# EtherealEngine/Universal-Volumetric

Measured on AMD Instinct MI355X. Metric: frames/s encode, 100k-vert mesh + 2048^2 texture, higher is better.
Workload: dtype u8/int32 (f32 only in the quantiser)

## Files before the change

universal-volumetric_amd/csrc/tex_device.hpp:

```cpp
#pragma once
#include <hip/hip_runtime.h>
#include <cstdint>
#include "tex_blocks.hpp"

#define TEX_MAX_LAYERS 64
#define TEX_MAX_CODEBOOK 16128
#define TEX_HS 64
#define TEX_VQ_ROUNDS 24
#define TEX_NMODEL 9
#define TEX_MODEL_CAP (TEX_MAX_CODEBOOK + TEX_HS + 8)
#define TEX_E_ALPHA (-60)

struct TexVQ {
  uint32_t n_items, K, nl, done, m_round, round_active;
  uint32_t *leaf;
  unsigned long long *stW, *stS, *stQ;
  uint8_t *splittable, *chosen; int32_t *axis; long long *th, *prio; uint32_t *newidx;
  uint32_t *split;
};

struct TexHuff { uint32_t n; uint32_t *freq; uint8_t *size; uint16_t *code; };

struct TexJob {
  const uint8_t *layer[TEX_MAX_LAYERS];
  uint32_t W, H, L, bx, by, nb, NB;
  uint32_t ashift;
  int32_t yflip; uint32_t Kmax_e, Kmax_s, T_skip;
  int32_t status;
  uint8_t *skip;
  uint32_t *cell;
  uint32_t *hist;
  uint8_t *flag; uint32_t *bsum;
  uint32_t ncell; uint32_t *cid, *cw, *cidx;
  TexVQ vq[2];
  uint32_t *ent;
  uint32_t *ecb; uint32_t ne; uint32_t *emap;
  uint16_t *bei, *bsi; uint32_t *bsel;
  uint32_t n_items; uint32_t *item;
  uint32_t *scb; uint8_t *sused; uint32_t *scu; uint32_t ns; uint32_t *smap;
  uint8_t *pred;
  uint32_t *clist; uint32_t ncoded[TEX_MAX_LAYERS];
  uint8_t *msym; uint32_t *gid, *gstart, *gsize;
  unsigned long long *tok;
  TexHuff hm[TEX_NMODEL];
  uint32_t *hscratch;
  uint8_t *sec[3]; uint32_t sec_cap[3], sec_len[3];
  uint8_t *slice[TEX_MAX_LAYERS]; uint32_t slice_cap, slice_len[TEX_MAX_LAYERS];
  unsigned long long pack_off, pack_len;
  unsigned long long slice_bits[TEX_MAX_LAYERS];
  uint32_t n_skipped;
};

__device__ inline void t_load_block(const TexJob &J, uint32_t l, uint32_t X, uint32_t Y, uint32_t px[16], uint32_t *amask = nullptr) {
  const uint8_t *img = J.layer[l >> J.ashift];
  const bool akind = (l & J.ashift) != 0;
  for (int y = 0; y < 4; y++) {
    uint32_t py = Y * 4 + y; if (py >= J.H) py = J.H - 1;
    const uint32_t sr = J.yflip ? J.H - 1 - py : py;
    const uint8_t *row = img + 4 * ((size_t)sr * J.W);
    if (X * 4 + 3 < J.W && (J.W & 3) == 0) {
      const uint4 v = *reinterpret_cast<const uint4 *>(row + 16 * (size_t)X);
      if (akind) { px[4 * y + 0] = (v.x >> 24) * 0x010101u; px[4 * y + 1] = (v.y >> 24) * 0x010101u; px[4 * y + 2] = (v.z >> 24) * 0x010101u; px[4 * y + 3] = (v.w >> 24) * 0x010101u; }
      else { px[4 * y + 0] = v.x & 0xffffffu; px[4 * y + 1] = v.y & 0xffffffu; px[4 * y + 2] = v.z & 0xffffffu; px[4 * y + 3] = v.w & 0xffffffu; }
      if (amask) *amask &= v.x & v.y & v.z & v.w;
    } else {
      for (int x = 0; x < 4; x++) { uint32_t pxx = X * 4 + x; if (pxx >= J.W) pxx = J.W - 1; const uint8_t *p = row + 4 * (size_t)pxx; px[4 * y + x] = akind ? (uint32_t)p[3] * 0x010101u : ((uint32_t)p[0] | ((uint32_t)p[1] << 8) | ((uint32_t)p[2] << 16)); if (amask) *amask &= (uint32_t)p[3] << 24; }
    }
  }
}

template <bool WANT_SEL, bool WANT_ROWS>
__device__ inline uint32_t t_eval_block(const uint32_t px[16], int c5r, int c5g, int c5b, int t, uint32_t *sel_out, unsigned long long *rows) {
  const int br = t_expand5(c5r), bg = t_expand5(c5g), bb = t_expand5(c5b);
  int cr[4], cg[4], cb[4];
  for (int s = 0; s < 4; s++) { const int d = t_inten(t, s); cr[s] = t_clampi(br + d, 0, 255); cg[s] = t_clampi(bg + d, 0, 255); cb[s] = t_clampi(bb + d, 0, 255); }
  uint32_t tot = 0, sel = 0;
  if (!WANT_ROWS) {
    const int d0 = t_inten(t, 0), d1 = t_inten(t, 1), d2 = t_inten(t, 2), d3 = t_inten(t, 3);
    const int lo = br < bg ? (br < bb ? br : bb) : (bg < bb ? bg : bb), hi = br > bg ? (br > bb ? br : bb) : (bg > bb ? bg : bb);
    if (!WANT_SEL && lo + d0 >= 0 && hi + d3 <= 255) {
      const int kh = 3 * d3 * d3, kl = 3 * d2 * d2;
      for (int i = 0; i < 16; i++) {
        const int er = br - (int)(px[i] & 255), eg = bg - (int)((px[i] >> 8) & 255), eb = bb - (int)((px[i] >> 16) & 255);
        const int A = er * er + eg * eg + eb * eb, B2 = 2 * (er + eg + eb), ab = B2 < 0 ? -B2 : B2;
        const int a = kh - d3 * ab, b = kl - d2 * ab;
        tot += (uint32_t)(A + (a < b ? a : b));
      }
      return tot;
    }
    if (lo + d0 >= 0 && hi + d3 <= 255) {
      const int k0 = 3 * d0 * d0, k1 = 3 * d1 * d1, k2 = 3 * d2 * d2, k3 = 3 * d3 * d3;
      for (int i = 0; i < 16; i++) {
        const int er = br - (int)(px[i] & 255), eg = bg - (int)((px[i] >> 8) & 255), eb = bb - (int)((px[i] >> 16) & 255);
        const int A = er * er + eg * eg + eb * eb, B2 = 2 * (er + eg + eb);
        const uint32_t e0 = (uint32_t)(A + d0 * B2 + k0), e1 = (uint32_t)(A + d1 * B2 + k1), e2 = (uint32_t)(A + d2 * B2 + k2), e3 = (uint32_t)(A + d3 * B2 + k3);
        uint32_t be = e0; int bs = 0;
        if (e1 < be) { be = e1; bs = 1; }
        if (e2 < be) { be = e2; bs = 2; }
        if (e3 < be) { be = e3; bs = 3; }
        tot += be; sel |= (uint32_t)bs << (2 * i);
      }
      if (WANT_SEL) *sel_out = sel;
      return tot;
    }
  }
  for (int i = 0; i < 16; i++) {
    const int r = (int)(px[i] & 255), g = (int)((px[i] >> 8) & 255), b = (int)((px[i] >> 16) & 255);
    uint32_t be = 0xffffffffu; int bs = 0; unsigned long long row = 0;
    for (int s = 0; s < 4; s++) {
      const int dr = cr[s] - r, dg = cg[s] - g, db = cb[s] - b;
      const uint32_t e = (uint32_t)(dr * dr + dg * dg + db * db);
      if (WANT_ROWS) row |= (unsigned long long)(e > 65535u ? 65535u : e) << (16 * s);
      if (e < be) { be = e; bs = s; }
    }
    tot += be; sel |= (uint32_t)bs << (2 * i);
    if (WANT_ROWS) rows[i] = row;
  }
  if (WANT_SEL) *sel_out = sel;
  return tot;
}

#ifdef HIPEMU
__device__ inline void t_mfma_i8_16x16x64(const uint32_t a[4], const uint32_t b[4], int acc[4]) {
  const int lane = hipemu_lane(), col = lane & 15, rg = lane >> 4;
  const unsigned long long a01 = a[0] | ((unsigned long long)a[1] << 32), a23 = a[2] | ((unsigned long long)a[3] << 32);
  const unsigned long long b01 = b[0] | ((unsigned long long)b[1] << 32), b23 = b[2] | ((unsigned long long)b[3] << 32);
  bool ok;
  for (int g = 0; g < 4; g++) {
    const unsigned long long B0 = hipemu_wave_exchange(b01, col + 16 * g, &ok), B1 = hipemu_wave_exchange(b23, col + 16 * g, &ok);
    for (int r = 0; r < 4; r++) {
      const unsigned long long A0 = hipemu_wave_exchange(a01, 4 * rg + r + 16 * g, &ok), A1 = hipemu_wave_exchange(a23, 4 * rg + r + 16 * g, &ok);
      int sum = 0;
      for (int j = 0; j < 8; j++) sum += (int)(int8_t)(A0 >> (8 * j)) * (int)(int8_t)(B0 >> (8 * j)) + (int)(int8_t)(A1 >> (8 * j)) * (int)(int8_t)(B1 >> (8 * j));
      acc[r] += sum;
    }
  }
}
#else
typedef int t_v4i __attribute__((ext_vector_type(4)));
__device__ __forceinline__ void t_mfma_i8_16x16x64(const uint32_t a[4], const uint32_t b[4], int acc[4]) {
  const t_v4i va = { (int)a[0], (int)a[1], (int)a[2], (int)a[3] }, vb = { (int)b[0], (int)b[1], (int)b[2], (int)b[3] }, vc = { acc[0], acc[1], acc[2], acc[3] };
  const t_v4i vd = __builtin_amdgcn_mfma_i32_16x16x64_i8(va, vb, vc, 0, 0, 0);
  acc[0] = vd.x; acc[1] = vd.y; acc[2] = vd.z; acc[3] = vd.w;
}
#endif

__device__ __forceinline__ void t_cell_coords(uint32_t cell, int x[4]) {
  x[0] = t_expand5((cell >> 10) & 31); x[1] = t_expand5((cell >> 5) & 31); x[2] = t_expand5(cell & 31); x[3] = t_inten((cell >> 15) & 7, 3);
}

struct TBitW { uint8_t *p; uint32_t cap, n; unsigned long long acc; int nacc; int overflow; };
__device__ inline void tb_init(TBitW &w, uint8_t *p, uint32_t cap) { w.p = p; w.cap = cap; w.n = 0; w.acc = 0; w.nacc = 0; w.overflow = 0; }
__device__ inline void tb_put(TBitW &w, uint32_t v, int n) {
  while (n > 0) {
    const int k = n > 24 ? 24 : n;
    w.acc |= (unsigned long long)(v & ((1u << k) - 1)) << w.nacc; w.nacc += k; v >>= k; n -= k;
    while (w.nacc >= 8) { if (w.n < w.cap) w.p[w.n] = (uint8_t)(w.acc & 0xff); else w.overflow = 1; w.n++; w.acc >>= 8; w.nacc -= 8; }
  }
}
__device__ inline void tb_flush(TBitW &w) { if (w.nacc > 0) { if (w.n < w.cap) w.p[w.n] = (uint8_t)(w.acc & 0xff); else w.overflow = 1; w.n++; w.acc = 0; w.nacc = 0; } }

__device__ __forceinline__ void t_vlc(uint32_t v, int cb, unsigned long long &bits, int &len) {
  bits = 0; len = 0;
  for (;;) { const uint32_t chunk = v & ((1u << cb) - 1); v >>= cb; bits |= (unsigned long long)(chunk | (v ? (1u << cb) : 0u)) << len; len += cb + 1; if (!v) break; }
}
```

universal-volumetric_amd/csrc/tex_encode.hip:

```cpp
#include "uvol_common.hpp"
#include "tex_device.hpp"
#include <algorithm>

#define TJOB_OR_RETURN TexJob &J = job[blockIdx.z]; if (J.status != 0) return
#define TEX_RETRY_ALPHA (~(size_t)0)

__device__ inline uint32_t t_block_excl_scan(uint32_t v, uint32_t *total) {
  __shared__ uint32_t wsum[UVOL_BLOCK / 64];
  const int lane = threadIdx.x & 63, w = threadIdx.x >> 6;
  uint32_t x = v;
  for (int d = 1; d < 64; d <<= 1) { uint32_t y = __shfl_up(x, d); if (lane >= d) x += y; }
  if (lane == 63) wsum[w] = x;
  __syncthreads();
  uint32_t base = 0, tot = 0;
  for (int i = 0; i < UVOL_BLOCK / 64; i++) { if (i < w) base += wsum[i]; tot += wsum[i]; }
  __syncthreads();
  *total = tot;
  return base + x - v;
}
__global__ void __launch_bounds__(UVOL_BLOCK) k_tscan_a(TexJob *job, uint32_t n) {
  TexJob &J = job[blockIdx.z];
  const uint32_t i = blockIdx.x * UVOL_BLOCK + threadIdx.x;
  uint32_t v = (J.status == 0 && i < n) ? J.flag[i] : 0, tot;
  t_block_excl_scan(v, &tot);
  if (threadIdx.x == 0) J.bsum[blockIdx.x] = tot;
}
__global__ void __launch_bounds__(UVOL_BLOCK) k_tscan_b(TexJob *job, uint32_t nblocks) {
  TexJob &J = job[blockIdx.z];
  __shared__ uint32_t carry;
  if (threadIdx.x == 0) carry = 0;
  __syncthreads();
  for (uint32_t b0 = 0; b0 < nblocks; b0 += UVOL_BLOCK) {
    const uint32_t i = b0 + threadIdx.x;
    uint32_t v = i < nblocks ? J.bsum[i] : 0, tot;
    const uint32_t ex = t_block_excl_scan(v, &tot);
    const uint32_t c = carry;
    if (i < nblocks) J.bsum[i] = c + ex;
    __syncthreads();
    if (threadIdx.x == 0) carry = c + tot;
    __syncthreads();
  }
  if (threadIdx.x == 0) J.bsum[nblocks] = carry;
}

__global__ void __launch_bounds__(UVOL_BLOCK) k_tex_skip(TexJob *job) {
  TJOB_OR_RETURN;
  const uint32_t b = blockIdx.x * UVOL_BLOCK + threadIdx.x;
  if (b >= J.nb) return;
  const uint32_t X = b % J.bx, Y = b / J.bx;
  uint32_t anchor[16], cur[16], amask = 0xff000000u;
  const uint32_t st = 1u << J.ashift;
  for (uint32_t kind = 0; kind < st; kind++) {
    t_load_block(J, kind, X, Y, anchor, &amask);
    J.skip[(size_t)kind * J.nb + b] = 0; J.flag[(size_t)kind * J.nb + b] = 1;
    for (uint32_t l = kind + st; l < J.L; l += st) {
      t_load_block(J, l, X, Y, cur, &amask);
      uint32_t d = 0;
      for (int i = 0; i < 16; i++) {
        const int dr = (int)(cur[i] & 255) - (int)(anchor[i] & 255), dg = (int)((cur[i] >> 8) & 255) - (int)((anchor[i] >> 8) & 255), db = (int)((cur[i] >> 16) & 255) - (int)((anchor[i] >> 16) & 255);
        d += (uint32_t)(dr * dr + dg * dg + db * db);
      }
      const bool sk = d <= J.T_skip;
      J.skip[(size_t)l * J.nb + b] = sk ? 1 : 0; J.flag[(size_t)l * J.nb + b] = sk ? 0 : 1;
      if (!sk) for (int i = 0; i < 16; i++) anchor[i] = cur[i];
    }
  }
  if (!J.ashift && (amask & 0xff000000u) != 0xff000000u) J.status = TEX_E_ALPHA;
}

__global__ void __launch_bounds__(UVOL_BLOCK) k_tex_fit(TexJob *job) {
  TJOB_OR_RETURN;
  const uint32_t it = blockIdx.x * UVOL_BLOCK + threadIdx.x;
  if (it >= J.n_items) return;
  const uint32_t b = J.item[it];
  const uint32_t l = b / J.nb, r = b % J.nb;
  uint32_t px[16]; t_load_block(J, l, r % J.bx, r / J.bx, px);
  int sum[3] = {0, 0, 0};
  for (int i = 0; i < 16; i++) { sum[0] += (int)(px[i] & 255); sum[1] += (int)((px[i] >> 8) & 255); sum[2] += (int)((px[i] >> 16) & 255); }
  int base5[3]; for (int c = 0; c < 3; c++) base5[c] = (((sum[c] + 8) >> 4) * 31 + 127) / 255;
  uint32_t best = 0xffffffffu; int bc0 = 0, bc1 = 0, bc2 = 0, bt = 0;
  for (int t = 0; t < 8; t++) for (int di = 0; di < 3; di++) {
    const int dd = di == 0 ? 0 : (di == 1 ? -1 : 1);
    const int c0 = t_clampi(base5[0] + dd, 0, 31), c1 = t_clampi(base5[1] + dd, 0, 31), c2 = t_clampi(base5[2] + dd, 0, 31);
    const uint32_t e = t_eval_block<false, false>(px, c0, c1, c2, t, nullptr, nullptr);
    if (e < best) { best = e; bt = t; bc0 = c0; bc1 = c1; bc2 = c2; }
  }
  for (int c = 0; c < 3; c++) for (int di = 1; di < 3; di++) {
    const int dd = di == 1 ? -1 : 1;
    int c0 = bc0 + (c == 0 ? dd : 0), c1 = bc1 + (c == 1 ? dd : 0), c2 = bc2 + (c == 2 ? dd : 0);
    const int cc = c == 0 ? c0 : (c == 1 ? c1 : c2);
    if (cc < 0 || cc > 31) continue;
    const uint32_t e = t_eval_block<false, false>(px, c0, c1, c2, bt, nullptr, nullptr);
    if (e < best) { best = e; bc0 = c0; bc1 = c1; bc2 = c2; }
  }
  const uint32_t cell = ((uint32_t)bt << 15) | ((uint32_t)bc0 << 10) | ((uint32_t)bc1 << 5) | (uint32_t)bc2;
  J.cell[b] = cell;
  atomicAdd(&J.hist[cell], 1u);
}

__global__ void __launch_bounds__(UVOL_BLOCK) k_cell_flags(TexJob *job) {
  TJOB_OR_RETURN;
  const uint32_t c = blockIdx.x * UVOL_BLOCK + threadIdx.x;
  if (c < (1u << 18)) J.flag[c] = J.hist[c] ? 1 : 0;
}
__global__ void __launch_bounds__(UVOL_BLOCK) k_cell_compact(TexJob *job) {
  TexJob &J = job[blockIdx.z];
  const uint32_t c = blockIdx.x * UVOL_BLOCK + threadIdx.x;
  const bool live = J.status == 0 && c < (1u << 18);
  uint32_t v = live ? J.flag[c] : 0, tot;
  const uint32_t pos = t_block_excl_scan(v, &tot) + J.bsum[blockIdx.x];
  if (live && v) { J.cid[pos] = c; J.cw[pos] = J.hist[c]; J.cidx[c] = pos; }
  if (blockIdx.x == 0 && threadIdx.x == 0 && J.status == 0) {
    const uint32_t n = J.bsum[(1u << 18) / UVOL_BLOCK];
    J.ncell = n;
    TexVQ &V = J.vq[0]; V.n_items = n; V.K = n < J.Kmax_e ? n : J.Kmax_e; V.nl = 1; V.done = (V.K <= 1) ? 1 : 0;
  }
}

template <int DIM> __device__ __forceinline__ void vq_item(const TexJob &J, uint32_t i, int x[DIM], unsigned long long &w) {
  if (DIM == 4) { t_cell_coords(J.cid[i], x); w = J.cw[i]; }
  else { const uint32_t s = J.bsel[J.item[i]]; for (int k = 0; k < DIM; k++) x[k] = (int)((s >> (2 * k)) & 3); w = 1; }
}
template <int DIM> __device__ __forceinline__ int vq_wd(int d) { return (DIM == 4 && d == 3) ? 2 : 1; }

template <int DIM>
__global__ void __launch_bounds__(UVOL_BLOCK) k_vq_zero(TexJob *job, int force) {
  TJOB_OR_RETURN;
  TexVQ &V = J.vq[DIM == 4 ? 0 : 1];
  if (V.done && !force) return;
  const uint32_t i = blockIdx.x * UVOL_BLOCK + threadIdx.x;
  if (i < V.K) V.stW[i] = 0;
  if (i < V.K * DIM) { V.stS[i] = 0; V.stQ[i] = 0; }
}
template <int DIM, int LCAP, typename CT>
__global__ void __launch_bounds__(UVOL_BLOCK) k_vq_stats(TexJob *job, int force, uint32_t leaf_base, uint32_t lds_leaves) {
  TJOB_OR_RETURN;
  TexVQ &V = J.vq[DIM == 4 ? 0 : 1];
  if ((V.done && !force) || V.nl <= leaf_base) return;
  UVOL_DYN_SMEM(CT, lds);
  const uint32_t nl = V.nl - leaf_base, pass = nl < (uint32_t)LCAP ? nl : (uint32_t)LCAP, ncap = pass < lds_leaves ? pass : lds_leaves, stride = 1 + 2 * DIM;
  for (uint32_t k = threadIdx.x; k < ncap * stride; k += UVOL_BLOCK) lds[k] = 0;
  __syncthreads();
  for (uint32_t base = blockIdx.x * UVOL_BLOCK; base < V.n_items; base += gridDim.x * UVOL_BLOCK) {
    const uint32_t i = base + threadIdx.x;
    const bool todo = i < V.n_items;
    const uint32_t l = todo ? V.leaf[i] : 0xffffffffu;
    if (!todo || l < leaf_base || l - leaf_base >= pass) continue;
    int x[DIM]; unsigned long long w; vq_item<DIM>(J, i, x, w);
    if (l - leaf_base >= ncap) {
      atomicAdd(&V.stW[l], w);
      for (int d = 0; d < DIM; d++) { atomicAdd(&V.stS[(size_t)l * DIM + d], w * (unsigned long long)x[d]); atomicAdd(&V.stQ[(size_t)l * DIM + d], w * (unsigned long long)(x[d] * x[d])); }
      continue;
    }
    CT *p = lds + (size_t)(l - leaf_base) * stride;
    atomicAdd(&p[0], (CT)w);
    for (int d = 0; d < DIM; d++) { atomicAdd(&p[1 + d], (CT)(w * (unsigned long long)x[d])); atomicAdd(&p[1 + DIM + d], (CT)(w * (unsigned long long)(x[d] * x[d]))); }
  }
  __syncthreads();
  for (uint32_t k = threadIdx.x; k < ncap * stride; k += UVOL_BLOCK) {
    const unsigned long long v = (unsigned long long)lds[k]; if (!v) continue;
    const uint32_t l = leaf_base + k / stride, f = k % stride;
    if (f == 0) atomicAdd(&V.stW[l], v);
    else if (f <= (uint32_t)DIM) atomicAdd(&V.stS[(size_t)l * DIM + (f - 1)], v);
    else atomicAdd(&V.stQ[(size_t)l * DIM + (f - 1 - DIM)], v);
  }
}
#define SEL_ILP 4
template <typename WT> __device__ __forceinline__ void sel_stats_accumulate(WT *lds, bool todo, uint32_t rl, uint32_t sw, uint32_t lane) {
  constexpr int QS = sizeof(WT) * 4;
  unsigned long long rem = __ballot(todo);
  for (int rounds = 0; rounds < 4 && rem; rounds++) {
    const uint32_t leader = (uint32_t)(__ffsll((long long)rem) - 1);
    const uint32_t ll = UVOL_READLANE(rl, leader);
    const bool inm = todo && rl == ll;
    const unsigned long long m = __ballot(inm);
    if (__popcll(m) < 24) break;
    WT myv = 0;
    for (int d = 0; d < 16; d++) {
      const uint32_t xv = (sw >> (2 * d)) & 3u;
      const uint32_t c1 = (uint32_t)__popcll(__ballot(inm && xv == 1)), c2 = (uint32_t)__popcll(__ballot(inm && xv == 2)), c3 = (uint32_t)__popcll(__ballot(inm && xv == 3));
      if (lane == (uint32_t)d) myv = (WT)(c1 + 2 * c2 + 3 * c3) | ((WT)(c1 + 4 * c2 + 9 * c3) << QS);
    }
    if (lane == 16) myv = (WT)__popcll(m);
    if (lane < 17 && myv) atomicAdd(&lds[ll * 17 + lane], myv);
    rem &= ~m;
    if (inm) todo = false;
  }
  if (!todo) return;
  WT *p = lds + (size_t)rl * 17;
  uint32_t f = lane % 17u;
  for (int k = 0; k < 17; k++) {
    const uint32_t xv = (sw >> (2 * (f & 15u))) & 3u;
    const WT v = f == 16u ? (WT)1 : ((WT)xv | ((WT)(xv * xv) << QS));
    if (v) atomicAdd(&p[f], v);
    f = f == 16u ? 0u : f + 1u;
  }
}
template <typename WT> __device__ __forceinline__ void sel_stats_flush(TexVQ &V, const WT *lds, uint32_t ncap, uint32_t leaf0) {
  constexpr int QS = sizeof(WT) * 4;
  const WT lo = ((WT)1 << QS) - 1;
  for (uint32_t k = threadIdx.x; k < ncap * 17; k += UVOL_BLOCK) {
    const WT v = lds[k]; if (!v) continue;
    const uint32_t l = leaf0 + k / 17, w = k % 17;
    if (w == 16) atomicAdd(&V.stW[l], (unsigned long long)v);
    else {
      if (v & lo) atomicAdd(&V.stS[(size_t)l * 16 + w], (unsigned long long)(v & lo));
      if (v >> QS) atomicAdd(&V.stQ[(size_t)l * 16 + w], (unsigned long long)(v >> QS));
    }
  }
}
template <typename WT> __global__ void __launch_bounds__(UVOL_BLOCK) k_sel_stats(TexJob *job, int force, uint32_t lcap, uint32_t leaf_base) {
  TJOB_OR_RETURN;
  TexVQ &V = J.vq[1];
  if ((V.done && !force) || V.nl <= leaf_base) return;
  UVOL_DYN_SMEM(WT, lds);
  const uint32_t nl = V.nl - leaf_base, ncap = nl < lcap ? nl : lcap;
  for (uint32_t k = threadIdx.x; k < ncap * 17; k += UVOL_BLOCK) lds[k] = 0;
  __syncthreads();
  const uint32_t lane = threadIdx.x & 63, n_items = V.n_items;
  const uint32_t *const leaf = V.leaf, *const item = J.item, *const bsel = J.bsel;
  for (uint32_t base = blockIdx.x * (UVOL_BLOCK * SEL_ILP); base < n_items; base += gridDim.x * (UVOL_BLOCK * SEL_ILP)) {
    uint32_t l[SEL_ILP], it[SEL_ILP], sw[SEL_ILP];
#pragma unroll
    for (int k = 0; k < SEL_ILP; k++) { const uint32_t i = base + k * UVOL_BLOCK + threadIdx.x; const bool in = i < n_items; l[k] = in ? leaf[i] : 0xffffffffu; it[k] = in ? item[i] : 0u; }
#pragma unroll
    for (int k = 0; k < SEL_ILP; k++) sw[k] = l[k] != 0xffffffffu ? bsel[it[k]] : 0u;
#pragma unroll
    for (int k = 0; k < SEL_ILP; k++) sel_stats_accumulate(lds, l[k] != 0xffffffffu && l[k] - leaf_base < ncap, l[k] - leaf_base, sw[k], lane);
  }
  __syncthreads();
  sel_stats_flush(V, lds, ncap, leaf_base);
}
template <typename WT> __global__ void __launch_bounds__(UVOL_BLOCK) k_sel_split_stats(TexJob *job, uint32_t lcap, uint32_t win_base) {
  TJOB_OR_RETURN;
  TexVQ &V = J.vq[1];
  if (!V.round_active || V.m_round <= win_base) return;
  UVOL_DYN_SMEM(WT, lds);
  const uint32_t m = V.m_round - win_base, ncap = m < lcap ? m : lcap, nl_old = V.nl - V.m_round, leaf0 = nl_old + win_base;
  for (uint32_t k = threadIdx.x; k < ncap * 17; k += UVOL_BLOCK) lds[k] = 0;
  __syncthreads();
  const uint32_t lane = threadIdx.x & 63, n_items = V.n_items;
  uint32_t *const leaf = V.leaf; const uint32_t *const split = V.split, *const item = J.item, *const bsel = J.bsel;
  for (uint32_t base = blockIdx.x * (UVOL_BLOCK * SEL_ILP); base < n_items; base += gridDim.x * (UVOL_BLOCK * SEL_ILP)) {
    uint32_t l[SEL_ILP], it[SEL_ILP], sw[SEL_ILP], sp[SEL_ILP];
#pragma unroll
    for (int k = 0; k < SEL_ILP; k++) { const uint32_t i = base + k * UVOL_BLOCK + threadIdx.x; const bool in = i < n_items; l[k] = in ? leaf[i] : 0xffffffffu; it[k] = in ? item[i] : 0u; }
#pragma unroll
    for (int k = 0; k < SEL_ILP; k++) { sw[k] = l[k] != 0xffffffffu ? bsel[it[k]] : 0u; sp[k] = (win_base == 0 && l[k] < nl_old) ? split[l[k]] : 0u; }
#pragma unroll
    for (int k = 0; k < SEL_ILP; k++) {
      bool todo = false; uint32_t nl_ = l[k];
      if (win_base == 0) {
        if ((sp[k] >> 31) && ((sw[k] >> (2 * ((sp[k] >> 24) & 15u))) & 3u) > ((sp[k] >> 16) & 0xffu)) { nl_ = sp[k] & 0xffffu; leaf[base + k * UVOL_BLOCK + threadIdx.x] = nl_; todo = true; }
      } else todo = l[k] != 0xffffffffu && l[k] >= leaf0;
      todo = todo && nl_ - leaf0 < ncap;
      sel_stats_accumulate(lds, todo, nl_ - leaf0, sw[k], lane);
    }
  }
  __syncthreads();
  sel_stats_flush(V, lds, ncap, leaf0);
}
template <int DIM, bool INCR>
__global__ void __launch_bounds__(UVOL_BLOCK) k_vq_decide(TexJob *job, int fold_only) {
  TJOB_OR_RETURN;
  TexVQ &V = J.vq[DIM == 4 ? 0 : 1];
  if (INCR && V.round_active) {
    const uint32_t nlp = V.nl - V.m_round;
    for (uint32_t l = threadIdx.x; l < nlp; l += UVOL_BLOCK) {
      if (!V.chosen[l]) continue;
      const uint32_t ch = V.newidx[l];
      V.stW[l] -= V.stW[ch];
      for (int d = 0; d < DIM; d++) { V.stS[(size_t)l * DIM + d] -= V.stS[(size_t)ch * DIM + d]; V.stQ[(size_t)l * DIM + d] -= V.stQ[(size_t)ch * DIM + d]; }
    }
    __syncthreads();
  }
  if (V.done || fold_only) { __syncthreads(); if (threadIdx.x == 0) V.round_active = 0; return; }
  const uint32_t nl = V.nl, K = V.K;
  __shared__ uint32_t s_navail, s_carry;
  if (threadIdx.x == 0) { s_navail = 0; s_carry = 0; }
  __syncthreads();
  uint32_t mine = 0;
  for (uint32_t l = threadIdx.x; l < nl; l += UVOL_BLOCK) {
    const long long W = (long long)V.stW[l]; long long D = 0, best = -1; int ax = 0;
    for (int d = 0; d < DIM; d++) {
      const long long S = (long long)V.stS[(size_t)l * DIM + d], Q = (long long)V.stQ[(size_t)l * DIM + d];
      const long long num = (W * Q - S * S) * vq_wd<DIM>(d);
      D += num; if (num > best) { best = num; ax = d; }
    }
    const uint8_t sp = D > 0 ? 1 : 0;
    V.splittable[l] = sp; V.axis[l] = ax; V.th[l] = W ? (long long)V.stS[(size_t)l * DIM + ax] / W : 0; V.prio[l] = W ? D / W : 0;
    mine += sp;
  }
  if (mine) atomicAdd(&s_navail, mine);
  __syncthreads();
  const uint32_t navail = s_navail;
  if (navail == 0) { if (threadIdx.x == 0) { V.done = 1; V.round_active = 0; } return; }
  const uint32_t room = K - nl, m = navail < room ? navail : room;
  for (uint32_t l = threadIdx.x; l < nl; l += UVOL_BLOCK) {
    uint8_t ch = V.splittable[l];
    if (ch && navail > room) {
      const long long p = V.prio[l]; uint32_t rank = 0;
      for (uint32_t j = 0; j < nl; j++) if (V.splittable[j]) { const long long pj = V.prio[j]; rank += (pj > p || (pj == p && j < l)) ? 1u : 0u; }
      ch = rank < m ? 1 : 0;
    }
    V.chosen[l] = ch;
  }
  __syncthreads();
  for (uint32_t b0 = 0; b0 < nl; b0 += UVOL_BLOCK) {
    const uint32_t l = b0 + threadIdx.x;
    uint32_t v = l < nl ? V.chosen[l] : 0, tot;
    const uint32_t ex = t_block_excl_scan(v, &tot);
    const uint32_t c = s_carry;
    if (l < nl) { V.newidx[l] = nl + c + ex; if (INCR) V.split[l] = v ? (0x80000000u | ((uint32_t)V.axis[l] << 24) | ((uint32_t)V.th[l] << 16) | (nl + c + ex)) : 0u; }
    __syncthreads();
    if (threadIdx.x == 0) s_carry = c + tot;
    __syncthreads();
  }
  if (threadIdx.x == 0) { V.m_round = m; V.round_active = 1; V.nl = nl + m; if (nl + m >= K) V.done = 1; }
  if (!INCR) for (uint32_t i = threadIdx.x; i < K * DIM; i += UVOL_BLOCK) { if (i < K) V.stW[i] = 0; V.stS[i] = 0; V.stQ[i] = 0; }
}
template <int DIM>
__global__ void __launch_bounds__(UVOL_BLOCK) k_vq_apply(TexJob *job) {
  TJOB_OR_RETURN;
  TexVQ &V = J.vq[DIM == 4 ? 0 : 1];
  if (!V.round_active) return;
  const uint32_t i = blockIdx.x * UVOL_BLOCK + threadIdx.x;
  if (i >= V.n_items) return;
  const uint32_t l = V.leaf[i];
  if (V.chosen[l]) {
    int x[DIM]; unsigned long long w; vq_item<DIM>(J, i, x, w);
    const int ax = V.axis[l];
    int xv = 0; for (int d = 0; d < DIM; d++) xv = d == ax ? x[d] : xv;
    if ((long long)xv > V.th[l]) V.leaf[i] = V.newidx[l];
  }
}
__global__ void __launch_bounds__(UVOL_BLOCK) k_ep_entries(TexJob *job) {
  TJOB_OR_RETURN;
  TexVQ &V = J.vq[0];
  const uint32_t k = blockIdx.x * UVOL_BLOCK + threadIdx.x;
  if (k >= V.nl) return;
  const long long W = (long long)V.stW[k]; if (!W) return;
  int c5[3];
  for (int d = 0; d < 3; d++) { const int m8 = (int)((2 * (long long)V.stS[(size_t)k * 4 + d] + W) / (2 * W)); c5[d] = t_clampi((m8 * 31 + 127) / 255, 0, 31); }
  const int mi = (int)((2 * (long long)V.stS[(size_t)k * 4 + 3] + W) / (2 * W));
  int bt = 0, bd = 1 << 30;
  for (int t = 0; t < 8; t++) { int d = t_inten(t, 3) - mi; d = d < 0 ? -d : d; if (d < bd) { bd = d; bt = t; } }
  J.ent[k] = ((uint32_t)bt << 15) | ((uint32_t)c5[0] << 10) | ((uint32_t)c5[1] << 5) | (uint32_t)c5[2];
}
__global__ void __launch_bounds__(UVOL_BLOCK) k_ep_assign(TexJob *job) {
  TJOB_OR_RETURN;
  TexVQ &V = J.vq[0];
  __shared__ int se[UVOL_BLOCK * 4];
  const uint32_t i = blockIdx.x * UVOL_BLOCK + threadIdx.x;
  const bool live = i < V.n_items;
  int x[4] = {0, 0, 0, 0}; if (live) t_cell_coords(J.cid[i], x);
  int bd = 0x7fffffff; uint32_t bk = 0;
  for (uint32_t k0 = 0; k0 < V.nl; k0 += UVOL_BLOCK) {
    __syncthreads();
    if (k0 + threadIdx.x < V.nl) { int e[4]; t_cell_coords(J.ent[k0 + threadIdx.x], e); for (int d = 0; d < 4; d++) se[threadIdx.x * 4 + d] = e[d]; }
    __syncthreads();
    const uint32_t kn = V.nl - k0 < UVOL_BLOCK ? V.nl - k0 : UVOL_BLOCK;
    if (live) for (uint32_t k = 0; k < kn; k++) {
      const int d0 = x[0] - se[k * 4], d1 = x[1] - se[k * 4 + 1], d2 = x[2] - se[k * 4 + 2], d3 = x[3] - se[k * 4 + 3];
      const int dist = d0 * d0 + d1 * d1 + d2 * d2 + 2 * d3 * d3;
      if (dist < bd) { bd = dist; bk = k0 + k; }
    }
  }
  if (live) V.leaf[i] = bk;
}

__global__ void __launch_bounds__(UVOL_BLOCK) k_unique(TexJob *job, int which) {
  TJOB_OR_RETURN;
  const uint32_t K = J.vq[which].nl;
  const uint32_t *val = which == 0 ? J.ent : J.scb;
  uint32_t *outv = which == 0 ? J.ecb : J.scu, *map = which == 0 ? J.emap : J.smap;
  uint8_t *first = J.vq[which].splittable;
  __shared__ uint32_t s_cnt;
  if (threadIdx.x == 0) s_cnt = 0;
  __syncthreads();
  for (uint32_t k = threadIdx.x; k < K; k += UVOL_BLOCK) {
    const bool used = which == 0 ? (J.vq[0].stW[k] != 0) : (J.sused[k] != 0);
    uint8_t f = 0;
    if (used) { f = 1; const uint32_t v = val[k]; for (uint32_t j = 0; j < k; j++) { const bool uj = which == 0 ? (J.vq[0].stW[j] != 0) : (J.sused[j] != 0); if (uj && val[j] == v) { f = 2; break; } } }
    first[k] = f;
  }
  __syncthreads();
  uint32_t mine = 0;
  for (uint32_t k = threadIdx.x; k < K; k += UVOL_BLOCK) {
    if (!first[k]) { map[k] = 0; continue; }
    const uint32_t v = val[k]; uint32_t less = 0;
    for (uint32_t j = 0; j < K; j++) less += (first[j] == 1 && val[j] < v) ? 1u : 0u;
    map[k] = less;
    if (first[k] == 1) { outv[less] = v; mine++; }
  }
  if (mine) atomicAdd(&s_cnt, mine);
  __syncthreads();
  if (threadIdx.x == 0) { if (which == 0) J.ne = s_cnt; else J.ns = s_cnt; }
}
// ... 992 lines not shown
```

Baseline: 3506.

## Restructure ETC1 cell fit with precomputed sums, udot4/sad intrinsics and uniform-block path

Replaces the per-candidate block evaluation in the texture fit kernel with an algebraic form. Per-block sums and squared norms are precomputed once per base colour, and the fast path uses a hinge-sum formula. It uses the udot4 and sad_u16 intrinsics for the per-pixel dot products and absolute differences. Uniform-colour blocks take a single-pixel template (N=1) that is scaled by 16. The old non-selector fast path in t_eval_block is removed. This adds more code, possible divergence between the N=1 and N=16 paths, and a risk of tie-breaking differences against the old search order.

```diff
diff --git a/universal-volumetric_amd/csrc/tex_device.hpp b/universal-volumetric_amd/csrc/tex_device.hpp
--- a/universal-volumetric_amd/csrc/tex_device.hpp
+++ b/universal-volumetric_amd/csrc/tex_device.hpp
@@ -78,16 +78,6 @@
   if (!WANT_ROWS) {
     const int d0 = t_inten(t, 0), d1 = t_inten(t, 1), d2 = t_inten(t, 2), d3 = t_inten(t, 3);
     const int lo = br < bg ? (br < bb ? br : bb) : (bg < bb ? bg : bb), hi = br > bg ? (br > bb ? br : bb) : (bg > bb ? bg : bb);
-    if (!WANT_SEL && lo + d0 >= 0 && hi + d3 <= 255) {
-      const int kh = 3 * d3 * d3, kl = 3 * d2 * d2;
-      for (int i = 0; i < 16; i++) {
-        const int er = br - (int)(px[i] & 255), eg = bg - (int)((px[i] >> 8) & 255), eb = bb - (int)((px[i] >> 16) & 255);
-        const int A = er * er + eg * eg + eb * eb, B2 = 2 * (er + eg + eb), ab = B2 < 0 ? -B2 : B2;
-        const int a = kh - d3 * ab, b = kl - d2 * ab;
-        tot += (uint32_t)(A + (a < b ? a : b));
-      }
-      return tot;
-    }
     if (lo + d0 >= 0 && hi + d3 <= 255) {
       const int k0 = 3 * d0 * d0, k1 = 3 * d1 * d1, k2 = 3 * d2 * d2, k3 = 3 * d3 * d3;
       for (int i = 0; i < 16; i++) {
@@ -121,6 +111,88 @@
 }
 
 #ifdef HIPEMU
+__device__ inline uint32_t t_absdiff(uint32_t a, uint32_t b) { return a > b ? a - b : b - a; }
+__device__ inline uint32_t t_udot4(uint32_t a, uint32_t b, uint32_t c) { for (int k = 0; k < 32; k += 8) c += ((a >> k) & 255u) * ((b >> k) & 255u); return c; }
+#else
+__device__ __forceinline__ uint32_t t_absdiff(uint32_t a, uint32_t b) { return __builtin_amdgcn_sad_u16(a, b, 0u); }
+__device__ __forceinline__ uint32_t t_udot4(uint32_t a, uint32_t b, uint32_t c) { return __builtin_amdgcn_udot4(a, b, c, false); }
+#endif
+template <int N>
+__device__ __forceinline__ int t_fit_sum_a(const int S[3], int Q, int br, int bg, int bb) {
+  return N * (br * br + bg * bg + bb * bb) - 2 * (br * S[0] + bg * S[1] + bb * S[2]) + Q;
+}
+template <int N>
+__device__ __forceinline__ uint32_t t_fit_abs_b(const uint32_t px[N], int br, int bg, int bb, uint32_t ab2[N]) {
+  uint32_t sum = 0;
+  for (int i = 0; i < N; i++) { ab2[i] = t_absdiff((uint32_t)(2 * (br + bg + bb)), t_udot4(px[i], 0x020202u, 0)); sum += ab2[i]; }
+  return sum & 0xffffu;
+}
+template <int N>
+__device__ inline int t_fit_eval(const uint32_t px[N], const uint32_t ab2[N], uint32_t sab2, int sa, int br, int bg, int bb, int t) {
+  const int S = etc1_mag_s(t), L = etc1_mag_l(t);
+  const int lo = br < bg ? (br < bb ? br : bb) : (bg < bb ? bg : bb), hi = br > bg ? (br > bb ? br : bb) : (bg > bb ? bg : bb);
+  if (lo - L >= 0 && hi + L <= 255) {
+    const uint32_t T = (uint32_t)(3 * (L + S));
+    uint32_t over = 0;
+    for (int i = 0; i < N; i++) over += ab2[i] > T ? ab2[i] - T : 0u;
+    return sa - (S * (int)sab2 - N * 3 * S * S + (L - S) * (int)(over & 0xffffu));
+  }
+  const int base[3] = { br, bg, bb };
+  int K[4]; uint32_t W[4];
+  for (int s = 0; s < 4; s++) {
+    const int d = s == 0 ? -L : (s == 1 ? -S : (s == 2 ? S : L));
+    K[s] = 0; W[s] = 0;
+    for (int c = 0; c < 3; c++) { const int col = t_clampi(base[c] + d, 0, 255); K[s] += (col - base[c]) * (col + base[c]); W[s] |= t_absdiff((uint32_t)col, (uint32_t)base[c]) << (8 * c); }
+  }
+  int acc = sa;
+  for (int i = 0; i < N; i++) {
+    const int g0 = K[0] + (int)(t_udot4(px[i], W[0], 0) << 1), g1 = K[1] + (int)(t_udot4(px[i], W[1], 0) << 1);
+    const int n2 = (int)(t_udot4(px[i], W[2], 0) << 1) - K[2], n3 = (int)(t_udot4(px[i], W[3], 0) << 1) - K[3];
+    const int m01 = g0 < g1 ? g0 : g1, m23 = -(n2 > n3 ? n2 : n3);
+    acc += m01 < m23 ? m01 : m23;
+  }
+  return acc;
+}
+template <int N>
+__device__ inline uint32_t t_fit_cell(const uint32_t *px) {
+  const int M = 16 / N;
+  int S[3] = { 0, 0, 0 }, Q = 0; uint32_t ab2[N];
+  for (int i = 0; i < N; i++) {
+    S[0] += (int)(px[i] & 255); S[1] += (int)((px[i] >> 8) & 255); S[2] += (int)((px[i] >> 16) & 255);
+    Q = (int)t_udot4(px[i], px[i], (uint32_t)Q);
+  }
+  int base5[3]; for (int c = 0; c < 3; c++) base5[c] = (((M * S[c] + 8) >> 4) * 31 + 127) / 255;
+  uint32_t key = 0xffffffffu;
+#pragma unroll 1
+  for (int di = 0; di < 3; di++) {
+    const int dd = di == 0 ? 0 : (di == 1 ? -1 : 1);
+    const int br = t_expand5(t_clampi(base5[0] + dd, 0, 31)), bg = t_expand5(t_clampi(base5[1] + dd, 0, 31)), bb = t_expand5(t_clampi(base5[2] + dd, 0, 31));
+    const int sa = t_fit_sum_a<N>(S, Q, br, bg, bb);
+    const uint32_t sab2 = t_fit_abs_b<N>(px, br, bg, bb, ab2);
+#pragma unroll 1
+    for (int t = 0; t < 8; t++) {
+      const uint32_t k = ((uint32_t)(M * t_fit_eval<N>(px, ab2, sab2, sa, br, bg, bb, t)) << 5) | (uint32_t)(3 * t + di);
+      key = k < key ? k : key;
+    }
+  }
+  const int bt = (int)(key & 31u) / 3, bdi = (int)(key & 31u) - 3 * bt, bdd = bdi == 0 ? 0 : (bdi == 1 ? -1 : 1);
+  uint32_t best = key >> 5;
+  int bc0 = t_clampi(base5[0] + bdd, 0, 31), bc1 = t_clampi(base5[1] + bdd, 0, 31), bc2 = t_clampi(base5[2] + bdd, 0, 31);
+#pragma unroll 1
+  for (int k = 0; k < 6; k++) {
+    const int c = k >> 1, dd = (k & 1) ? 1 : -1;
+    const int c0 = bc0 + (c == 0 ? dd : 0), c1 = bc1 + (c == 1 ? dd : 0), c2 = bc2 + (c == 2 ? dd : 0);
+    const int cc = c == 0 ? c0 : (c == 1 ? c1 : c2);
+    if (cc < 0 || cc > 31) continue;
+    const int br = t_expand5(c0), bg = t_expand5(c1), bb = t_expand5(c2);
+    const uint32_t sab2 = t_fit_abs_b<N>(px, br, bg, bb, ab2);
+    const uint32_t e = (uint32_t)(M * t_fit_eval<N>(px, ab2, sab2, t_fit_sum_a<N>(S, Q, br, bg, bb), br, bg, bb, bt));
+    if (e < best) { best = e; bc0 = c0; bc1 = c1; bc2 = c2; }
+  }
+  return ((uint32_t)bt << 15) | ((uint32_t)bc0 << 10) | ((uint32_t)bc1 << 5) | (uint32_t)bc2;
+}
+
+#ifdef HIPEMU
 __device__ inline void t_mfma_i8_16x16x64(const uint32_t a[4], const uint32_t b[4], int acc[4]) {
   const int lane = hipemu_lane(), col = lane & 15, rg = lane >> 4;
   const unsigned long long a01 = a[0] | ((unsigned long long)a[1] << 32), a23 = a[2] | ((unsigned long long)a[3] << 32);
diff --git a/universal-volumetric_amd/csrc/tex_encode.hip b/universal-volumetric_amd/csrc/tex_encode.hip
--- a/universal-volumetric_amd/csrc/tex_encode.hip
+++ b/universal-volumetric_amd/csrc/tex_encode.hip
@@ -75,25 +75,10 @@
   const uint32_t b = J.item[it];
   const uint32_t l = b / J.nb, r = b % J.nb;
   uint32_t px[16]; t_load_block(J, l, r % J.bx, r / J.bx, px);
-  int sum[3] = {0, 0, 0};
-  for (int i = 0; i < 16; i++) { sum[0] += (int)(px[i] & 255); sum[1] += (int)((px[i] >> 8) & 255); sum[2] += (int)((px[i] >> 16) & 255); }
-  int base5[3]; for (int c = 0; c < 3; c++) base5[c] = (((sum[c] + 8) >> 4) * 31 + 127) / 255;
-  uint32_t best = 0xffffffffu; int bc0 = 0, bc1 = 0, bc2 = 0, bt = 0;
-  for (int t = 0; t < 8; t++) for (int di = 0; di < 3; di++) {
-    const int dd = di == 0 ? 0 : (di == 1 ? -1 : 1);
-    const int c0 = t_clampi(base5[0] + dd, 0, 31), c1 = t_clampi(base5[1] + dd, 0, 31), c2 = t_clampi(base5[2] + dd, 0, 31);
-    const uint32_t e = t_eval_block<false, false>(px, c0, c1, c2, t, nullptr, nullptr);
-    if (e < best) { best = e; bt = t; bc0 = c0; bc1 = c1; bc2 = c2; }
-  }
-  for (int c = 0; c < 3; c++) for (int di = 1; di < 3; di++) {
-    const int dd = di == 1 ? -1 : 1;
-    int c0 = bc0 + (c == 0 ? dd : 0), c1 = bc1 + (c == 1 ? dd : 0), c2 = bc2 + (c == 2 ? dd : 0);
-    const int cc = c == 0 ? c0 : (c == 1 ? c1 : c2);
-    if (cc < 0 || cc > 31) continue;
-    const uint32_t e = t_eval_block<false, false>(px, c0, c1, c2, bt, nullptr, nullptr);
-    if (e < best) { best = e; bc0 = c0; bc1 = c1; bc2 = c2; }
-  }
-  const uint32_t cell = ((uint32_t)bt << 15) | ((uint32_t)bc0 << 10) | ((uint32_t)bc1 << 5) | (uint32_t)bc2;
+  uint32_t diff = 0;
+  for (int i = 1; i < 16; i++) diff |= px[i] ^ px[0];
+  uint32_t cell;
+  if (diff) cell = t_fit_cell<16>(px); else cell = t_fit_cell<1>(px);
   J.cell[b] = cell;
   atomicAdd(&J.hist[cell], 1u);
 }
```

Result: no change. 3488 (-0.5%).
